# HiLab-git/FPL-plus

Hardware: AMD Instinct MI355X
Metric: 3D volumes/sec (train step, 80x160x160) (higher is better)
Workload: dtype bf16; 1 GPU; UNet3D-DSBN 32-base-ch bf16 (fp32 master weights), per-GPU batch 2x1x80x160x160 synthetic VS crops, DiceLoss + Adam, domain alternating per step; global_batch=2, parallelism=dp1, step=zero_grad+forward+loss+backward+allreduce+adam

## Files before the change

### fpl-plus_amd/csrc/common.h

```cpp
#pragma once
#include <hip/hip_runtime.h>
#include <stdint.h>
#include <stdio.h>
#include <stdarg.h>
#include <string.h>
#include "../../include/fplx.h"

typedef __bf16 bf16_t;

#define FPLX_WAVE 64

inline char* fplx_err_buf() {
  static thread_local char buf[512];
  return buf;
}
inline int fplx_fail(int code, const char* fmt, ...) {
  va_list ap;
  va_start(ap, fmt);
  vsnprintf(fplx_err_buf(), 512, fmt, ap);
  va_end(ap);
  return code;
}
inline int fplx_check_launch(const char* what) {
  hipError_t e = hipGetLastError();
// ... 59 lines not shown
}
struct FplxTileRange { int64_t first, end, step; };
__device__ __forceinline__ FplxTileRange fplx_xcd_tiles(int64_t ntiles, int on) {
  FplxTileRange t = {(int64_t)blockIdx.x, ntiles, (int64_t)gridDim.x};
  if (!on || gridDim.x < 16) return t;
  const unsigned c = blockIdx.x & 7u, xcd = (blockIdx.y * gridDim.x + blockIdx.x) & 7u;
  const int64_t q = ntiles >> 3, r = ntiles & 7;
  const int64_t start = xcd * q + ((int64_t)xcd < r ? xcd : r);
  t.first = start + (blockIdx.x >> 3);
  t.end = start + q + ((int64_t)xcd < r ? 1 : 0);
  t.step = (gridDim.x - c + 7u) >> 3;
  return t;
}
#endif
#define FPLX_KNOB_LIST(X)                                                                                              \
  X(XCD, "xcd", 1)                                                    \
  X(BRICK, "brick", 1)                                    \
  X(BRICK_FILL, "brick_fill", 192)           \
  X(BRICK_GEO, "brick_geo", -1)                    \
  X(BRICK_KSPLIT, "brick_ksplit", 0)                                             \
  X(EDGE_BLOCKS, "edge_blocks", 1024)                             \
  X(STEM_ROWS, "stem_rows", 1)                                              \
  X(OUTCONV_T, "outconv_t", 1)                                 \
  X(OUTCONV_DGRAD_MFMA, "outconv_dgrad_mfma", 1)                                                                       \
  X(OUTCONV_FWD_ROWS, "outconv_fwd_rows", 1)  \
  X(OUTCONV_DGRAD_ROWS, "outconv_dgrad_rows", 1)  \
  X(PACK_TILED, "pack_tiled", 1)                                                                                       \
  X(PACK_MULTI, "pack_multi", 1)                                                                                       \
  X(MARCH, "march", 1)                               \
  X(MARCH64_FW, "march64_fw", 0)                                \
  X(MARCH_DS, "march_ds", 0)                                       \
  X(MARCH128, "march128", 1)                                                                                           \
  X(MARCH64_LW, "march64_lw", 1)            \
  X(MARCH32_V2, "march32_v2", 4)              \
  X(WG_COT_MINVOX, "wg_cot_minvox", 0)                                                                                 \
  X(WG_TW, "wg_tw", 0)                                                                                                 \
  X(WG_CIT, "wg_cit", 2)                                                                                               \
  X(WG_COT, "wg_cot", 2)                                                                                               \
  X(WG_DS, "wg_ds", 0)                                                                                                 \
  X(WG_VOX, "wg_vox", 1)                              \
  X(WG_ROLL, "wg_roll", 1)                     \
  X(WG_ROLL_GEO, "wg_roll_geo", 0)          \
  X(WG_ROLL_M16, "wg_roll_m16", 1)                 \
  X(WG_ROLL_MB, "wg_roll_mb", 1)            \
  X(WG_ROLL_CUS, "wg_roll_cus", 256)                                \
  X(WG_ROLL_OVH, "wg_roll_ovh", 9)                     \
  X(WG_ROLL_MINVOX, "wg_roll_minvox", 0)                                                   \
  X(WG_ROLL2D, "wg_roll2d", 1)              \
  X(WG_ROLL2D_OVH, "wg_roll2d_ovh", 3)      \
  X(WG_REDUCE_ROWS, "wg_reduce_rows", 8)    \
  X(WG_VOX_LW, "wg_vox_lw", 1)              \
  X(WG_VOX_CUS, "wg_vox_cus", 128)          \
  X(WG_VOX_MAXV, "wg_vox_maxv", 10000)         \
  X(STREAM_MIN_W, "stream_min_w", 64)                                                                                  \
  X(TILE_MT, "tile_mt", 0)                                                                                             \
  X(TILE_NT, "tile_nt", 0)                                                                                             \
  X(TILE_KS, "tile_ks", 0)                                                                                             \
  X(MID_TILE, "mid_tile", 1)                                                                                           \
  X(DECONV_ROWS, "deconv_rows", 1)                                                                                     \
  X(DECONV_DGRAD_ROWS, "deconv_dgrad_rows", 1)   \
  X(ROWS_SMALL_DIV, "rows_small_div", 16)   \
  X(EW_GROUP, "ew_group", 1)                                                                                           \
  X(POOL_COL, "pool_col", 1)                         \
  X(EW_INFLIGHT, "ew_inflight", 2)          \
  X(EW_INFLIGHT_REDUCE, "ew_inflight_reduce", 2)
enum FplxKnobId {
#define FPLX_KNOB_ENUM(id, key, def) FPLX_K_##id,
  FPLX_KNOB_LIST(FPLX_KNOB_ENUM)
#undef FPLX_KNOB_ENUM
  FPLX_K_COUNT
};
extern "C" __attribute__((visibility("hidden"))) int64_t fplx_knob_values[FPLX_K_COUNT];
static inline int64_t fplx_knob(int id) { return __atomic_load_n(&fplx_knob_values[id], __ATOMIC_RELAXED); }
static inline int fplx_xcd_on() { return (int)fplx_knob(FPLX_K_XCD); }

static inline int fplx_rows_for(int64_t voxels) {
  constexpr int cap = 512;
  const int div = voxels <= 32768 ? (int)fplx_knob(FPLX_K_ROWS_SMALL_DIV) : 64;
  int64_t r = (voxels + div - 1) / div;
  if (r > cap) r = cap;
  if (r < 1) r = 1;
  return (int)r;
}
```

### fpl-plus_amd/csrc/conv_mfma.hip

```cpp
#include "common.h"
#include <stdlib.h>

namespace {

typedef __attribute__((ext_vector_type(8))) __bf16 bf16x8;
typedef __attribute__((ext_vector_type(16))) float f32x16;

constexpr int DIRECT_THREADS = 256;

template <int MT, int NTL, int MODE>
__global__ void __launch_bounds__(DIRECT_THREADS)
conv_fwd_direct(const bf16_t* __restrict__ x, int64_t ldx, const bf16_t* __restrict__ wp,
                const float* __restrict__ bias, bf16_t* __restrict__ y, int64_t ldy, int N, int D, int H, int W,
                int Cin, int Cout, float* __restrict__ stats, float* __restrict__ partial = nullptr) {
  const int lane = threadIdx.x & 63, wave = threadIdx.x >> 6;
  const int r = lane & 31, kh8 = (lane >> 5) * 8;
  const int64_t V = (int64_t)N * D * H * W;
  const int64_t m0 = ((int64_t)blockIdx.x * 4 + wave) * (MT * 32);
  const int n0 = blockIdx.y * (NTL * 32);

  int vn[MT], vd[MT], vh[MT], vw[MT];
  bool vok[MT];
#pragma unroll
  for (int t = 0; t < MT; ++t) {
// ... 714 lines not shown
#pragma unroll
        for (int g4 = 0; g4 < 4; ++g4)
          *reinterpret_cast<float4*>(out + (tap * 32 + co) * 32 + 8 * g4 + rbase) =
              make_float4(acc[o * 7 + i][4 * g4 + 0], acc[o * 7 + i][4 * g4 + 1], acc[o * 7 + i][4 * g4 + 2],
                          acc[o * 7 + i][4 * g4 + 3]);
      }
    }
  }
}

template <int COT>
__global__ void __launch_bounds__(256)
conv_wgrad_vox(const bf16_t* __restrict__ x, int64_t ldx, const bf16_t* __restrict__ dy, int64_t ldy,
               float* __restrict__ part, int Cin, int Cout, VoxGeo g, int xcd) {
  const FplxBlock bid = fplx_xcd_block(xcd);
  switch (__builtin_amdgcn_readfirstlane(threadIdx.x >> 6)) {
    case 0: wgrad_vox_march<0, COT>(x, ldx, dy, ldy, part, Cin, Cout, g, bid); break;
    case 1: wgrad_vox_march<1, COT>(x, ldx, dy, ldy, part, Cin, Cout, g, bid); break;
    case 2: wgrad_vox_march<2, COT>(x, ldx, dy, ldy, part, Cin, Cout, g, bid); break;
    default: wgrad_vox_march<3, COT>(x, ldx, dy, ldy, part, Cin, Cout, g, bid); break;
  }
}

template <int WV, int SL>
__device__ __forceinline__ void wgrad_vox_lw_chunk(f32x16 (&acc)[7], const char* const (&xb)[7], const char* dyb, const char* mkb) {
  using L = VXL<1>;
  constexpr int NT = (27 - WV + 3) / 4, NKS = VX_KC / 16, NI = NKS * NT;
  constexpr int XOFF = SL * L::X_SLOT, DOFF = SL * L::DY_SLOT, MOFF = SL * L::MK_SLOT;
  constexpr int PD = 3, RING = PD + 1;
  bf16x8 fbw[2], far[RING];
  u32x4v mkr[RING];
  auto masked = [](int j) { const int tap = WV + 4 * j; return ((tap / 3) % 3) != 1 || (tap % 3) != 1; };
  auto load_item = [&](int t) {
    const int ks = t / NT, j = t % NT, tap = WV + 4 * j;
    far[t % RING] = tr_frag(xb[j] + XOFF + ks * 1024);
    if (masked(j)) mkr[t % RING] = *reinterpret_cast<const u32x4v*>(mkb + MOFF + ((tap % 9) * 16 + 2 * ks) * 16);
  };
  fbw[0] = tr_frag(dyb + DOFF);
#pragma unroll
  for (int t = 0; t < PD; ++t) load_item(t);
#pragma unroll
  for (int t = 0; t < NI; ++t) {
    const int ks = t / NT, j = t % NT;
    if (t + PD < NI) load_item(t + PD);
    if (j == 0 && ks + 1 < NKS) fbw[(ks + 1) & 1] = tr_frag(dyb + DOFF + (ks + 1) * 1024);
    __builtin_amdgcn_sched_barrier(0);
    bf16x8 a = far[t % RING];
    if (masked(j)) a = __builtin_bit_cast(bf16x8, __builtin_bit_cast(u32x4v, a) & mkr[t % RING]);
    acc[j] = __builtin_amdgcn_mfma_f32_32x32x16_bf16(a, fbw[ks & 1], acc[j], 0, 0, 0);
    __builtin_amdgcn_sched_barrier(0);
  }
}

template <int WV>
__device__ __forceinline__ void wgrad_vox_lw_compute(float* __restrict__ part, int Cin, int Cout, const VoxGeo& g, const FplxBlock& bid,
                                                     char* smem, int lane, int k0, int k1) {
  using L = VXL<1>;
  const int W = g.W, XR = VX_KC + 2 * W + 2, xplane = XR * 64;
  const int gq = lane >> 4, q = (lane & 15) >> 2, pp = lane & 3;
  const int lane_off = (8 * (gq >> 1) + q) * 64 + (16 * (gq & 1) + 4 * pp) * 2;
  constexpr int NT = (27 - WV + 3) / 4;
  const char* xb[7];
#pragma unroll
  for (int j = 0; j < 7; ++j) {
    const int tap = j < NT ? WV + 4 * j : WV;
    const int kd = tap / 9, kh = (tap / 3) % 3, kw = tap % 3;
    xb[j] = smem + L::X0 + kd * xplane + (kh * W + kw) * 64 + lane_off;
  }
  const char* dyb = smem + L::DY0 + lane_off;
  const char* mkb = smem + L::MK0 + (gq >> 1) * 16;
  f32x16 acc[7];
#pragma unroll
  for (int i = 0; i < 7; ++i)
#pragma unroll
    for (int r = 0; r < 16; ++r) acc[i][r] = 0.f;
  asm volatile("s_waitcnt lgkmcnt(0)\n\ts_barrier" ::: "memory");
  for (int kc = k0;;) {
    wgrad_vox_lw_chunk<WV, 0>(acc, xb, dyb, mkb);
    asm volatile("s_waitcnt lgkmcnt(0)\n\ts_barrier" ::: "memory");
    kc += VX_KC;
    if (kc >= k1) break;
    wgrad_vox_lw_chunk<WV, 1>(acc, xb, dyb, mkb);
    asm volatile("s_waitcnt lgkmcnt(0)\n\ts_barrier" ::: "memory");
    kc += VX_KC;
    if (kc >= k1) break;
  }
  const int ncit = Cin / 32;
  const int cot = bid.y / ncit, cit = bid.y % ncit;
  const int co = lane & 31, rbase = (lane >> 5) * 4;
  const int pair = cot * ncit + cit;
  float* out = part + ((int64_t)bid.x * (ncit * (Cout / 32)) + pair) * (27 * 1024);
#pragma unroll
  for (int i = 0; i < 7; ++i) {
    const int tap = WV + 4 * i;
    if (tap < 27) {
#pragma unroll
      for (int g4 = 0; g4 < 4; ++g4)
        *reinterpret_cast<float4*>(out + (tap * 32 + co) * 32 + 8 * g4 + rbase) =
            make_float4(acc[i][4 * g4 + 0], acc[i][4 * g4 + 1], acc[i][4 * g4 + 2], acc[i][4 * g4 + 3]);
    }
  }
}

__global__ void __launch_bounds__(512)
conv_wgrad_vox_lw(const bf16_t* __restrict__ x, int64_t ldx, const bf16_t* __restrict__ dy, int64_t ldy,
                  float* __restrict__ part, int Cin, int Cout, const VoxGeo g, int xcd) {
  using L = VXL<1>;
  extern __shared__ __attribute__((aligned(16))) char smem[];
  const FplxBlock bid = fplx_xcd_block(xcd);
  const int W = g.W, HW = g.HW, V = g.V;
  const int XR = VX_KC + 2 * W + 2;
  unsigned char* vc = reinterpret_cast<unsigned char*>(smem + L::VC0);
  const int tid = threadIdx.x, lane = tid & 63;
  const int wave8 = __builtin_amdgcn_readfirstlane(tid >> 6);
  const int ncit = Cin / 32;
  const int cot = bid.y / ncit, cit = bid.y % ncit;
  const int k0 = bid.x * g.kper;
  const int k1 = (k0 + g.kper < V) ? k0 + g.kper : V;
  const int halo = HW + W + 1;
  const int tb0 = k0 - halo, tbn = (k1 - k0 + VX_KC - 1) / VX_KC * VX_KC + 2 * halo;
  for (int t = tid; t < tbn; t += 512) {
    const int u = tb0 + t;
    unsigned char c = 0xFF;
    if (u >= 0 && u < V) {
      const unsigned q1 = __umulhi((unsigned)u, g.mW), w_ = (unsigned)u - q1 * (unsigned)W;
      const unsigned q2 = __umulhi(q1, g.mH), h_ = q1 - q2 * (unsigned)g.H;
      const unsigned q3 = __umulhi(q2, g.mD), d_ = q2 - q3 * (unsigned)g.D;
      c = (unsigned char)((d_ == 0 ? 1 : 0) | (d_ == (unsigned)g.D - 1 ? 2 : 0) | (h_ == 0 ? 4 : 0) |
                          (h_ == (unsigned)g.H - 1 ? 8 : 0) | (w_ == 0 ? 16 : 0) | (w_ == (unsigned)W - 1 ? 32 : 0));
    }
    vc[t] = c;
  }
  __syncthreads();
  if (wave8 < 4) {
    switch (wave8) {
      case 0: wgrad_vox_lw_compute<0>(part, Cin, Cout, g, bid, smem, lane, k0, k1); break;
      case 1: wgrad_vox_lw_compute<1>(part, Cin, Cout, g, bid, smem, lane, k0, k1); break;
      case 2: wgrad_vox_lw_compute<2>(part, Cin, Cout, g, bid, smem, lane, k0, k1); break;
      default: wgrad_vox_lw_compute<3>(part, Cin, Cout, g, bid, smem, lane, k0, k1); break;
    }
    return;
  }
  const int lw = wave8 - 4;
  const bf16_t* xg = x + cit * 32;
  const bf16_t* dyg = dy + cot * 32;
  u32x4v rx, ry;
  rx[0] = __builtin_amdgcn_readfirstlane((unsigned)(size_t)xg);
  rx[1] = __builtin_amdgcn_readfirstlane((unsigned)((size_t)xg >> 32) & 0xFFFFu);
  rx[2] = __builtin_amdgcn_readfirstlane((unsigned)((int64_t)V * ldx * 2));
  rx[3] = 0x00020000u;
  ry[0] = __builtin_amdgcn_readfirstlane((unsigned)(size_t)dyg);
  ry[1] = __builtin_amdgcn_readfirstlane((unsigned)((size_t)dyg >> 32) & 0xFFFFu);
  ry[2] = __builtin_amdgcn_readfirstlane((unsigned)((int64_t)V * ldy * 2));
  ry[3] = 0x00020000u;
  const unsigned lds0 = __builtin_amdgcn_readfirstlane((unsigned)(size_t)((__attribute__((address_space(3))) char*)smem));
  auto buf_dma = [&](const u32x4v& rsrc, unsigned vo, unsigned dst_off) {
    const unsigned dst = lds0 + dst_off;
    unsigned keep;
    asm volatile("s_mov_b32 %0, m0\n\ts_mov_b32 m0, %4\n\ts_nop 0\n\tbuffer_load_dwordx4 %1, %2, %3 offen lds\n\ts_mov_b32 m0, %0"
                 : "=&s"(keep) : "v"(vo), "s"(rsrc), "s"(0u), "s"(dst) : "memory");
  };
  const int nxp = (3 * XR + 15) / 16;
  auto stage = [&](int kn, int slot) {
    for (int p = lw; p < nxp + VX_KC / 16; p += 4) {
      if (p < nxp) {
        const int rr = p * 16 + (lane >> 2);
        const int pl = (rr >= XR ? 1 : 0) + (rr >= 2 * XR ? 1 : 0), row = rr - pl * XR;
        const int u = kn + row - (W + 1) + (pl - 1) * HW;
        const int t = u - tb0;
        const bool in = t >= 0 && t < tbn;
        const unsigned c = vc[in ? t : 0];
        const bool ok = in && c != 0xFFu && !((pl == 0 && (c & 2u)) || (pl == 2 && (c & 1u)));
        const unsigned vo = ok ? (unsigned)(((int64_t)u * ldx + (lane & 3) * 8) * 2) : 0x80000000u;
        if (rr < 3 * XR) buf_dma(rx, vo, (unsigned)(L::X0 + slot * L::X_SLOT + p * 1024));
      } else {
        const int v_ = kn + (p - nxp) * 16 + (lane >> 2);
        const unsigned vo = v_ < k1 ? (unsigned)(((int64_t)v_ * ldy + (lane & 3) * 8) * 2) : 0x80000000u;
        buf_dma(ry, vo, (unsigned)(L::DY0 + slot * L::DY_SLOT + (p - nxp) * 1024));
      }
    }
    if (lw < 2) {
      const unsigned c = vc[kn - tb0 + lw * 64 + lane];
      const uint64_t h0 = __ballot(c & 4), h2 = __ballot(c & 8), w0 = __ballot(c & 16), w2 = __ballot(c & 32);
      char* mk_n = smem + L::MK0 + slot * L::MK_SLOT;
#pragma unroll
      for (int rnd = 0; rnd < 2; ++rnd) {
        const int e = rnd * 64 + lane;
        if (e < 72) {
          const int combo = e >> 3, jj = e & 7, kh = combo / 3, kw = combo - 3 * kh;
          const uint64_t inv = (kh == 0 ? h0 : (kh == 2 ? h2 : 0)) | (kw == 0 ? w0 : (kw == 2 ? w2 : 0));
          const unsigned by = (unsigned)(inv >> (8 * jj)) & 0xFFu;
          u32x4v m_;
#pragma unroll
          for (int q_ = 0; q_ < 4; ++q_)
            m_[q_] = ((by >> (2 * q_)) & 1u ? 0u : 0xFFFFu) | ((by >> (2 * q_ + 1)) & 1u ? 0u : 0xFFFF0000u);
          *reinterpret_cast<u32x4v*>(mk_n + (combo * 16 + lw * 8 + jj) * 16) = m_;
        }
      }
    }
  };
  stage(k0, 0);
  asm volatile("s_waitcnt vmcnt(0)" ::: "memory");
  asm volatile("s_waitcnt lgkmcnt(0)\n\ts_barrier" ::: "memory");
  for (int kc = k0, slot = 0;; slot ^= 1) {
    const int kn = kc + VX_KC;
    if (kn < k1) stage(kn, slot ^ 1);
    asm volatile("s_waitcnt vmcnt(0)" ::: "memory");
    asm volatile("s_waitcnt lgkmcnt(0)\n\ts_barrier" ::: "memory");
    kc = kn;
    if (kc >= k1) break;
  }
}

struct VoxCfg { int ok, cot, npairs; VoxGeo g; size_t ws, lds; };
inline VoxCfg vox_cfg(int n, int d, int h, int w, int cin, int cout) {
  VoxCfg c = {};
  const int64_t V = (int64_t)n * d * h * w;
  const int mode = (int)fplx_knob(FPLX_K_WG_VOX);
  if (!mode || cin % 32 != 0 || cout % 32 != 0 || w > VX_MAXW || w < 2 || h < 2 || d < 2 || V >= ((int64_t)1 << 24)) return c;
  if (mode == 1 && V > (int64_t)fplx_knob(FPLX_K_WG_VOX_MAXV)) return c;
  const int lwk = (int)fplx_knob(FPLX_K_WG_VOX_LW);
  const bool lw = lwk == 2 || (lwk == 1 && V <= 2048);
  c.cot = (cout % 64 == 0 && !lw) ? 2 : 1;
  c.npairs = (cin / 32) * (cout / 32);
  const int groups = c.npairs / c.cot;
  const int chunks = (int)((V + VX_KC - 1) / VX_KC);
  const int cus = (int)fplx_knob(FPLX_K_WG_VOX_CUS);
  int S = (cus + groups - 1) / groups;
  if (S > chunks) S = chunks;
  if (S < 1) S = 1;
  const int cper = (chunks + S - 1) / S;
  S = (chunks + cper - 1) / cper;
  VoxGeo& g = c.g;
  g.V = (int)V; g.D = d; g.H = h; g.W = w; g.HW = h * w;
  g.mW = (unsigned)((((uint64_t)1 << 32) + w - 1) / w);
  g.mH = (unsigned)((((uint64_t)1 << 32) + h - 1) / h);
  g.mD = (unsigned)((((uint64_t)1 << 32) + d - 1) / d);
  g.kper = cper * VX_KC; g.S = S;
  c.ws = (size_t)S * c.npairs * 27 * 1024 * sizeof(float);
  c.lds = (size_t)(c.cot == 2 ? VXL<2>::VC0 : VXL<1>::VC0) + (size_t)(g.kper + 2 * (g.HW + w + 1)) + 16;
  c.lds = (c.lds + 15) / 16 * 16;
  if (c.lds > 160 * 1024) return c;
  c.ok = 1;
  return c;
}

__global__ void __launch_bounds__(DIRECT_THREADS)
deconv_fwd_mfma(const bf16_t* __restrict__ x, int64_t ldx, const bf16_t* __restrict__ wf,
                const float* __restrict__ bias, bf16_t* __restrict__ y, int64_t ldy, int N, int D, int H, int W,
                int Cin, int Cout, int sd, int vec_ok, int xcd) {
  const int lane = threadIdx.x & 63, wave = threadIdx.x >> 6;
  const int r = lane & 31, kh8 = (lane >> 5) * 8;
  const int64_t V = (int64_t)N * D * H * W;
  const FplxBlock bid = fplx_xcd_block(xcd);
  const int64_t m0 = ((int64_t)bid.x * 4 + wave) * 32;
  const int n0 = bid.y * 32, tap0 = bid.z * 4;
  const int64_t v = m0 + r;
  const bool ok = v < V;
  const bf16_t* ap = x + (ok ? v : 0) * ldx + kh8;
  const bf16x8 zero = {0, 0, 0, 0, 0, 0, 0, 0};
  f32x16 acc[4];
#pragma unroll
  for (int t = 0; t < 4; ++t)
#pragma unroll
// ... 233 lines not shown
  const int co = lane & 31, rbase = (lane >> 5) * 4;
#pragma unroll
  for (int t = 0; t < 2; ++t)
#pragma unroll
    for (int c = 0; c < CIT; ++c)
#pragma unroll
      for (int i = 0; i < 16; ++i) {
        const int ci = (i & 3) + 8 * (i >> 2) + rbase;
        out[(((2 * wave + t) * CIT + c) * 32 + ci) * 32 + co] = acc[t][c][i];
      }
  if (want_bias) {
    float* red = reinterpret_cast<float*>(smem);
#pragma unroll
    for (int j = 0; j < 8; ++j) red[tid * 8 + j] = bsum[j];
    __syncthreads();
    if (tid < 32) {
      const int cc = tid >> 3, j = tid & 7;
      float t = 0.f;
      for (int k = 0; k < 64; ++k) t += red[(k * 4 + cc) * 8 + j];
      bpart[(int64_t)blockIdx.x * Cout + cot * 32 + tid] = t;
    }
  }
}

__global__ void __launch_bounds__(64) deconv_bias_reduce(const float* __restrict__ bpart, int rows, int C, float* __restrict__ db) {
  const int c = blockIdx.x;
  float t = 0.f;
  for (int r = threadIdx.x; r < rows; r += 64) t += bpart[(int64_t)r * C + c];
  t = wave_sum(t);
  if (threadIdx.x == 0) db[c] = t;
}

__global__ void __launch_bounds__(256)
deconv_wgrad_reduce(const float* __restrict__ part, int nblk, int npairs, int cit, int Cin, int Cout,
                    float* __restrict__ dw, int ntaps) {
  __shared__ float red[256];
  const int64_t per = (int64_t)8 * cit * 1024, total = npairs * per;
  const int64_t i = (int64_t)blockIdx.x * 64 + (threadIdx.x & 63);
  const int pl = threadIdx.x >> 6, o = threadIdx.x & 63;
  float t = 0.f;
  if (i < total)
    for (int b = pl; b < nblk; b += 4) t += part[(int64_t)b * total + i];
  red[pl * 64 + o] = t;
  __syncthreads();
  if (pl != 0 || i >= total) return;
  t = red[o] + red[64 + o] + red[128 + o] + red[192 + o];
  const int co_l = i & 31, ci_l = (i >> 5) & 31, c = (int)((i >> 10) % cit), tap = (int)((i / (1024 * cit)) % 8);
  const int pair = (int)(i / per);
  const int ncig = Cin / (32 * cit);
  const int co = (pair / ncig) * 32 + co_l, ci = ((pair % ncig) * cit + c) * 32 + ci_l;
  if (tap < ntaps) dw[((int64_t)ci * Cout + co) * ntaps + tap] = t;
}

struct DwCfg { int cit, npairs, nblk; size_t ws; };
inline DwCfg dw_cfg(int n, int d, int h, int w, int cin, int cout) {
  DwCfg c;
  c.cit = (cin % 128 == 0) ? 4 : (cin % 64 == 0 ? 2 : 1);
  c.npairs = (cin / (32 * c.cit)) * (cout / 32);
  const int64_t chunks = ((int64_t)n * d * h * w + 127) / 128;
  int nb = 512 / c.npairs;
  if (nb < 1) nb = 1;
  if (nb > chunks) nb = (int)chunks;
  c.nblk = nb;
  c.ws = (size_t)c.nblk * c.npairs * 8 * c.cit * 1024 * sizeof(float) + (size_t)c.nblk * cout * sizeof(float);
  return c;
}

template <int CIN>
struct StreamGeo {
  static constexpr int ROWB = CIN * 2, CH = ROWB / 16;
  static constexpr int SW = 34, SH = 10, SLAB = SW * SH;
  static constexpr int GT = CIN == 32 ? 27 : 3, NG = 27 / GT;
  static constexpr int NSLOT = CIN == 32 ? 4 : 3, NWBUF = NG == 1 ? 1 : 2;
  static constexpr int SLAB_BYTES = SLAB * ROWB, WBUF_BYTES = GT * 32 * ROWB;
  static constexpr int NLD = (SLAB * CH + 255) / 256, NLW = NG == 1 ? 1 : (GT * 32 * CH + 255) / 256;
  static constexpr int LDS = NSLOT * SLAB_BYTES + NWBUF * WBUF_BYTES;
  static __device__ __forceinline__ int swz(int row) { return (row / (16 / CH)) % CH; }
};

template <int CIN>
__global__ void __launch_bounds__(256)
conv_fwd_stream(const bf16_t* __restrict__ x, int64_t ldx, const bf16_t* __restrict__ wp,
                const float* __restrict__ bias, bf16_t* __restrict__ y, int64_t ldy, int N, int D, int H, int W,
                int Cout, float* __restrict__ stats, int tilesH, int tilesW, int dsegs, int dlen) {
  typedef StreamGeo<CIN> G;
  extern __shared__ __attribute__((aligned(16))) char smem[];
  char* slabs = smem;
  char* wbuf = smem + G::NSLOT * G::SLAB_BYTES;
  const int tid = threadIdx.x, lane = tid & 63, wave = tid >> 6;
  const int r = lane & 31, khalf = lane >> 5;
  int b = blockIdx.x;
  const int seg = b % dsegs; b /= dsegs;
  const int tw = b % tilesW; b /= tilesW;
  const int th = b % tilesH; b /= tilesH;
  const int n = b;
  const int h0 = th * 8, w0 = tw * 32, d0 = seg * dlen;
  const int d1 = (d0 + dlen < D) ? d0 + dlen : D;
  const int n0 = blockIdx.y * 32;

  uint4 sreg[G::NLD], wreg[G::NLW];
  auto slab_fetch = [&](int d) {
    const bool dok = d >= 0 && d < D;
#pragma unroll
    for (int k = 0; k < G::NLD; ++k) {
      const int i = tid + k * 256;
      const int vox = i / G::CH, c = i % G::CH;
// ... 827 lines not shown
}
extern "C" int fplx_mfma_conv3d_fwd_act_cat2(const void* x0, const void* x1, int64_t ldx, const void* wp, const float* bias,
                                             const float* slope, void* y, int64_t ldy, int n, int d, int h, int w, int cin,
                                             int cout, int nmod0, hipStream_t st) {
  if (!fplx_mfma_conv3d_act_cat2_ok(n, d, h, w, cin, cout, 0) || !mfma_applicable(ldx, ldy, cin, cout, x0, y, wp)) return 0;
  int geo, ks, bricks;
  fplx_brick_plan(n, d, h, w, cin, cout, &geo, &ks, &bricks);
  return fplx_brick_conv3d_fwd_act(x0, ldx, wp, bias, y, ldy, n, d, h, w, cin, cout, nullptr, nullptr, geo, ks, st, slope, x1, nmod0);
}
extern "C" int fplx_mfma_conv3d_fwd_act(const void* x, int64_t ldx, const void* wp, const float* bias, const float* slope, void* y,
                                        int64_t ldy, int n, int d, int h, int w, int cin, int cout, void* ws, size_t ws_bytes,
                                        int mid, hipStream_t st) {
  return mfma_fwd_impl(x, ldx, wp, bias, y, ldy, n, d, h, w, cin, cout, nullptr, ws, ws_bytes, mid, st, slope);
}

extern "C" int fplx_wgroll_ok(int n, int d, int h, int w, int cin, int cout, int64_t ldx, int64_t ldy);
extern "C" size_t fplx_wgroll_ws_bytes(int n, int d, int h, int w, int cin, int cout);
extern "C" int fplx_wgroll_conv3d_wgrad(const void* x, int64_t ldx, const void* dy, int64_t ldy, float* dw, int n, int d, int h,
                                        int w, int cin, int cout, void* ws, size_t ws_bytes, hipStream_t st, const void* x1, int mid);
extern "C" int fplx_wgrad_reduce_launch(const float* part, int nblk, int npairs, int cin, int cout, float* dw, int mid,
                                        hipStream_t st) {
  const int64_t total = (int64_t)npairs * 27 * 1024;
  wgrad_finish(part, nblk, npairs, cin, cout, dw, mid, st);
  return fplx_check_launch("wgrad_stream_reduce");
}

extern "C" int fplx_mfma_conv3d_wgrad_cit(int n, int d, int h, int w, int cin, int cout) {
  if (cin % 32 != 0 || cout % 32 != 0) return 0;
  return wg_cfg(n, d, h, w, cin, cout).cit;
}

extern "C" size_t fplx_mfma_conv3d_wgrad_ws_bytes(int n, int d, int h, int w, int cin, int cout) {
  if (cin % 32 != 0 || cout % 32 != 0) return 0;
  const size_t a = wg_cfg(n, d, h, w, cin, cout).ws;
  const VoxCfg v = vox_cfg(n, d, h, w, cin, cout);
  size_t m = (v.ok && v.ws > a) ? v.ws : a;
  if (fplx_wgroll_ok(n, d, h, w, cin, cout, cin, cout)) { const size_t r = fplx_wgroll_ws_bytes(n, d, h, w, cin, cout); if (r > m) m = r; }
  return m;
}

extern "C" int fplx_mfma_conv3d_wgrad(const void* x, int64_t ldx, const void* dy, int64_t ldy, float* dw, int n, int d,
                                      int h, int w, int cin, int cout, void* ws, size_t ws_bytes, hipStream_t st,
                                      const void* x1, int mid) {
  if (cin % 32 != 0 || cout % 32 != 0 || ldx % 8 != 0 || ldy % 8 != 0 || ((uintptr_t)x % 16) || ((uintptr_t)dy % 16))
    return 0;
  if (!x1 && !mid) {
    const VoxCfg v = vox_cfg(n, d, h, w, cin, cout);
    if (v.ok) {
      if (ws_bytes < v.ws) return fplx_fail(FPLX_E_WORKSPACE, "mfma_conv3d_wgrad: workspace %zu < %zu", ws_bytes, v.ws);
      dim3 grid(v.g.S, v.npairs / v.cot);
      const int lwk = (int)fplx_knob(FPLX_K_WG_VOX_LW);
      if ((lwk == 2 || (lwk == 1 && v.g.V <= 2048)) && v.cot == 1 && (int64_t)v.g.V * ldx * 2 < ((int64_t)1 << 31) &&
          (int64_t)v.g.V * ldy * 2 < ((int64_t)1 << 31)) {
        (void)hipFuncSetAttribute((const void*)conv_wgrad_vox_lw, hipFuncAttributeMaxDynamicSharedMemorySize, (int)v.lds);
        conv_wgrad_vox_lw<<<grid, 512, v.lds, st>>>((const bf16_t*)x, ldx, (const bf16_t*)dy, ldy, (float*)ws, cin, cout, v.g, fplx_xcd_on());
      } else if (v.cot == 2) {
        (void)hipFuncSetAttribute((const void*)conv_wgrad_vox<2>, hipFuncAttributeMaxDynamicSharedMemorySize, (int)v.lds);
        conv_wgrad_vox<2><<<grid, 256, v.lds, st>>>((const bf16_t*)x, ldx, (const bf16_t*)dy, ldy, (float*)ws, cin, cout, v.g, fplx_xcd_on());
      } else {
        (void)hipFuncSetAttribute((const void*)conv_wgrad_vox<1>, hipFuncAttributeMaxDynamicSharedMemorySize, (int)v.lds);
        conv_wgrad_vox<1><<<grid, 256, v.lds, st>>>((const bf16_t*)x, ldx, (const bf16_t*)dy, ldy, (float*)ws, cin, cout, v.g, fplx_xcd_on());
      }
      wgrad_finish((const float*)ws, v.g.S, v.npairs, cin, cout, dw, 0, st);
      int rcv = fplx_check_launch("mfma_conv3d_wgrad_vox");
      return rcv < 0 ? rcv : 1;
    }
  }
  {
    const int rr = fplx_wgroll_conv3d_wgrad(x, ldx, dy, ldy, dw, n, d, h, w, cin, cout, ws, ws_bytes, st, x1, mid);
    if (rr != 0) return rr;
  }
  const WgCfg c = wg_cfg(n, d, h, w, cin, cout);
  if (x1 && (c.cit != 2 || cin != 64 || ((uintptr_t)x1 % 16))) return 0;
  if (ws_bytes < c.ws) return fplx_fail(FPLX_E_WORKSPACE, "mfma_conv3d_wgrad: workspace %zu < %zu", ws_bytes, c.ws);
  dim3 grid(c.nblk, c.npairs / (c.cit * c.cot));
#define LAUNCH_WG2(TW_, CIT_, COT_, TWOD_)                                                                          \
  do {                                                                                                              \
    const size_t lds = (size_t)(3 * CIT_ * (WG_TH + 2) * (TW_ + 2) + COT_ * WG_TH * TW_) * 64;                      \
    (void)hipFuncSetAttribute((const void*)conv_wgrad_stream<TW_, CIT_, COT_, TWOD_>, hipFuncAttributeMaxDynamicSharedMemorySize, (int)lds); \
    conv_wgrad_stream<TW_, CIT_, COT_, TWOD_><<<grid, 256, lds, st>>>((const bf16_t*)x, ldx, (const bf16_t*)dy, ldy, (float*)ws, n, d, \
                                                                h, w, cin, cout, c.tilesH, c.tilesW, c.dsegs, c.dlen, (const bf16_t*)x1, fplx_xcd_on()); \
  } while (0)
#define LAUNCH_WG(TW_, CIT_, COT_) do { if (mid) LAUNCH_WG2(TW_, CIT_, COT_, true); else LAUNCH_WG2(TW_, CIT_, COT_, false); } while (0)
  if (c.tw == 32) { if (c.cot == 2) LAUNCH_WG(32, 1, 2); else if (c.cit == 2) LAUNCH_WG(32, 2, 1); else LAUNCH_WG(32, 1, 1); }
  else { if (c.cot == 2) LAUNCH_WG(16, 1, 2); else if (c.cit == 2) LAUNCH_WG(16, 2, 1); else LAUNCH_WG(16, 1, 1); }
#undef LAUNCH_WG
#undef LAUNCH_WG2
  const int64_t total = (int64_t)c.npairs * 27 * 1024;
  wgrad_finish((const float*)ws, c.nblk, c.npairs, cin, cout, dw, mid, st);
  int rc = fplx_check_launch("mfma_conv3d_wgrad");
  return rc < 0 ? rc : 1;
}

extern "C" int fplx_mfma_deconv2_fwd(const void* x, int64_t ldx, const void* wf, const float* bias, void* y, int64_t ldy,
                                     int n, int d, int h, int w, int cin, int cout, int sd, hipStream_t st) {
  if (cin % 32 != 0 || cout % 32 != 0 || ldx % 8 != 0 || ((uintptr_t)x % 16) || ((uintptr_t)wf % 16)) return 0;
  const int64_t V = (int64_t)n * d * h * w;
  if (V >= ((int64_t)1 << 31)) return 0;
  const int vec_ok = ldy % 8 == 0 && ((uintptr_t)y % 16) == 0;
  {
    const int krows = (int)fplx_knob(FPLX_K_DECONV_ROWS);
    const int ks = cin / 16, ntc = cout / 32;
    if (krows && sd == 2 && vec_ok && V >= 32 * 1024 && ((ks == 4 && ntc == 1) || (ks == 8 && ntc == 2) || (ks == 8 && ntc == 1) ||
                                                         (ks == 4 && ntc == 2))) {
      const int64_t nt = (V + 31) / 32;
      const unsigned nb = (unsigned)(nt < 1024 ? nt : 1024);
#define LAUNCH_DR(KS_, NTC_) deconv_fwd_rows<KS_, NTC_><<<nb, 256, 0, st>>>((const bf16_t*)x, ldx, (const bf16_t*)wf, bias, \
                                                                           (bf16_t*)y, ldy, n, d, h, w, fplx_xcd_on())
// ... 34 lines not shown
  if (sd == 2 && fplx_knob(FPLX_K_DECONV_DGRAD_ROWS) && ((V + 127) / 128) * (cin / 64) < 128 && cin % 64 == 0 && cout % 16 == 0 &&
      ldx % 8 == 0 && ((uintptr_t)dx % 16) == 0) {
    dim3 gs((unsigned)((V + 31) / 32), cin / 64);
    deconv_dgrad_small<<<gs, 256, 0, st>>>((const bf16_t*)dy, ldy, (const bf16_t*)wb, (bf16_t*)dx, ldx, n, d, h, w, cout, cin);
    int rcs = fplx_check_launch("mfma_deconv2_dgrad_small");
    return rcs < 0 ? rcs : 1;
  }
#define LAUNCH_DD(MT_, NTL_, MODE_, GRID_)                                                                          \
  conv_fwd_direct<MT_, NTL_, MODE_><<<GRID_, DIRECT_THREADS, 0, st>>>((const bf16_t*)dy, ldy, (const bf16_t*)wb, nullptr, \
                                                                      (bf16_t*)dx, ldx, n, d, h, w, cout, cin, nullptr)
  if (cin % 64 == 0) {
    dim3 grid((unsigned)((V + 255) / 256), cin / 64);
    if ((int64_t)grid.x * grid.y < 192) {
      dim3 g1((unsigned)((V + 127) / 128), cin / 64);
      if (sd == 2) LAUNCH_DD(1, 2, 1, g1); else LAUNCH_DD(1, 2, 2, g1);
    } else if (sd == 2) LAUNCH_DD(2, 2, 1, grid);
    else LAUNCH_DD(2, 2, 2, grid);
  } else {
    dim3 grid((unsigned)((V + 511) / 512), cin / 32);
    if (sd == 2) LAUNCH_DD(4, 1, 1, grid); else LAUNCH_DD(4, 1, 2, grid);
  }
#undef LAUNCH_DD
  int rc = fplx_check_launch("mfma_deconv2_dgrad");
  return rc < 0 ? rc : 1;
}

extern "C" size_t fplx_mfma_deconv2_wgrad_ws_bytes(int n, int d, int h, int w, int cin, int cout) {
  if (cin % 32 != 0 || cout % 32 != 0) return 0;
  return dw_cfg(n, d, h, w, cin, cout).ws;
}

extern "C" int fplx_mfma_deconv2_wgrad(const void* x, int64_t ldx, const void* dy, int64_t ldy, float* dw, float* db,
                                       int n, int d, int h, int w, int cin, int cout, void* ws, size_t ws_bytes,
                                       int sd, hipStream_t st) {
  if (cin % 32 != 0 || cout % 32 != 0 || ldx % 8 != 0 || ldy % 8 != 0 || ((uintptr_t)x % 16) || ((uintptr_t)dy % 16))
    return 0;
  const DwCfg c = dw_cfg(n, d, h, w, cin, cout);
  if (ws_bytes < c.ws) return fplx_fail(FPLX_E_WORKSPACE, "mfma_deconv2_wgrad: workspace %zu < %zu", ws_bytes, c.ws);
  dim3 grid(c.nblk, c.npairs);
  const size_t lds = (size_t)(c.cit + 8) * 128 * 64;
  float* bpart = db ? (float*)((char*)ws + (size_t)c.nblk * c.npairs * 8 * c.cit * 1024 * sizeof(float)) : nullptr;
#define LAUNCH_DW(CIT)                                                                                              \
  do {                                                                                                              \
    (void)hipFuncSetAttribute((const void*)deconv_wgrad_mfma<CIT>, hipFuncAttributeMaxDynamicSharedMemorySize, (int)lds); \
    deconv_wgrad_mfma<CIT><<<grid, 256, lds, st>>>((const bf16_t*)x, ldx, (const bf16_t*)dy, ldy, (float*)ws, bpart, n, d, \
                                                   h, w, cin, cout, sd);                                            \
  } while (0)
  if (c.cit == 4) LAUNCH_DW(4);
  else if (c.cit == 2) LAUNCH_DW(2);
  else LAUNCH_DW(1);
#undef LAUNCH_DW
  const int64_t total = (int64_t)c.npairs * 8 * c.cit * 1024;
  if (db) deconv_bias_reduce<<<cout, 64, 0, st>>>(bpart, c.nblk, cout, db);
  deconv_wgrad_reduce<<<(unsigned)((total + 63) / 64), 256, 0, st>>>((const float*)ws, c.nblk, c.npairs, c.cit, cin, cout, dw,
                                                                      4 * sd);
  int rc = fplx_check_launch("mfma_deconv2_wgrad");
  return rc < 0 ? rc : 1;
}
```

Baseline: 246.9 volumes/s.

## Write vox wgrad directly to dw, add deep wgrad kernel and row-wise deconv reduce

When there is a single split (S==1), the lightweight vox wgrad kernel now transposes its accumulators through LDS and writes the final weight layout straight into dw. This skips the partial-buffer write and the separate wgrad_finish pass. A new 8-wave conv_wgrad_deep kernel for the cot==2 case is added behind knob level 2, so it is off by default. The deconv wgrad reduction is replaced by a row-per-block kernel that reduces float4 partials across blocks in LDS and writes coalesced rows. The cost is more LDS per block for the direct path, plus extra code complexity.

```diff
diff --git a/fpl-plus_amd/csrc/common.h b/fpl-plus_amd/csrc/common.h
--- a/fpl-plus_amd/csrc/common.h
+++ b/fpl-plus_amd/csrc/common.h
@@ -135,6 +135,7 @@
   X(WG_VOX_LW, "wg_vox_lw", 1)              \
   X(WG_VOX_CUS, "wg_vox_cus", 128)          \
   X(WG_VOX_MAXV, "wg_vox_maxv", 10000)         \
+  X(WG_DEEP, "wg_deep", 1)                  \
   X(STREAM_MIN_W, "stream_min_w", 64)                                                                                  \
   X(TILE_MT, "tile_mt", 0)                                                                                             \
   X(TILE_NT, "tile_nt", 0)                                                                                             \
diff --git a/fpl-plus_amd/csrc/conv_mfma.hip b/fpl-plus_amd/csrc/conv_mfma.hip
--- a/fpl-plus_amd/csrc/conv_mfma.hip
+++ b/fpl-plus_amd/csrc/conv_mfma.hip
@@ -790,7 +790,25 @@
   }
 }
 
-template <int WV>
+constexpr int VXD_TS = 1024 + 4;
+__device__ __forceinline__ void wgrad_vox_direct_copy(const char* smem, float* __restrict__ dw, int Cin, const FplxBlock& bid, int tid) {
+  const float* tile = reinterpret_cast<const float*>(smem);
+  const int ncit = Cin / 32;
+  const int cot = bid.y / ncit, cit = bid.y % ncit;
+  float* row0 = dw + ((int64_t)cot * 32 * Cin + cit * 32) * 27;
+#pragma unroll 1
+  for (int i = tid; i < 32 * 216; i += 512) {
+    const int row = i / 216, j = i - row * 216;
+    float v[4];
+#pragma unroll
+    for (int k = 0; k < 4; ++k) {
+      const int e = 4 * j + k, ci = e / 27, tap = e - 27 * ci;
+      v[k] = tile[tap * VXD_TS + row * 32 + ci];
+    }
+    *reinterpret_cast<float4*>(row0 + (int64_t)row * Cin * 27 + 4 * j) = make_float4(v[0], v[1], v[2], v[3]);
+  }
+}
+template <int WV, bool DIRECT>
 __device__ __forceinline__ void wgrad_vox_lw_compute(float* __restrict__ part, int Cin, int Cout, const VoxGeo& g, const FplxBlock& bid,
                                                      char* smem, int lane, int k0, int k1) {
   using L = VXL<1>;
@@ -823,6 +841,23 @@
     kc += VX_KC;
     if (kc >= k1) break;
   }
+  if constexpr (DIRECT) {
+    float* tile = reinterpret_cast<float*>(smem);
+    const int co = lane & 31, rbase = (lane >> 5) * 4;
+#pragma unroll
+    for (int i = 0; i < 7; ++i) {
+      const int tap = WV + 4 * i;
+      if (tap < 27) {
+#pragma unroll
+        for (int g4 = 0; g4 < 4; ++g4)
+          *reinterpret_cast<float4*>(tile + tap * VXD_TS + co * 32 + 8 * g4 + rbase) =
+              make_float4(acc[i][4 * g4 + 0], acc[i][4 * g4 + 1], acc[i][4 * g4 + 2], acc[i][4 * g4 + 3]);
+      }
+    }
+    asm volatile("s_waitcnt lgkmcnt(0)\n\ts_barrier" ::: "memory");
+    wgrad_vox_direct_copy(smem, part, Cin, bid, WV * 64 + lane);
+    return;
+  }
   const int ncit = Cin / 32;
   const int cot = bid.y / ncit, cit = bid.y % ncit;
   const int co = lane & 31, rbase = (lane >> 5) * 4;
@@ -840,6 +875,7 @@
   }
 }
 
+template <bool DIRECT>
 __global__ void __launch_bounds__(512)
 conv_wgrad_vox_lw(const bf16_t* __restrict__ x, int64_t ldx, const bf16_t* __restrict__ dy, int64_t ldy,
                   float* __restrict__ part, int Cin, int Cout, const VoxGeo g, int xcd) {
@@ -872,10 +908,10 @@
   __syncthreads();
   if (wave8 < 4) {
     switch (wave8) {
-      case 0: wgrad_vox_lw_compute<0>(part, Cin, Cout, g, bid, smem, lane, k0, k1); break;
-      case 1: wgrad_vox_lw_compute<1>(part, Cin, Cout, g, bid, smem, lane, k0, k1); break;
-      case 2: wgrad_vox_lw_compute<2>(part, Cin, Cout, g, bid, smem, lane, k0, k1); break;
-      default: wgrad_vox_lw_compute<3>(part, Cin, Cout, g, bid, smem, lane, k0, k1); break;
+      case 0: wgrad_vox_lw_compute<0, DIRECT>(part, Cin, Cout, g, bid, smem, lane, k0, k1); break;
+      case 1: wgrad_vox_lw_compute<1, DIRECT>(part, Cin, Cout, g, bid, smem, lane, k0, k1); break;
+      case 2: wgrad_vox_lw_compute<2, DIRECT>(part, Cin, Cout, g, bid, smem, lane, k0, k1); break;
+      default: wgrad_vox_lw_compute<3, DIRECT>(part, Cin, Cout, g, bid, smem, lane, k0, k1); break;
     }
     return;
   }
@@ -948,6 +984,208 @@
     kc = kn;
     if (kc >= k1) break;
   }
+  if constexpr (DIRECT) {
+    asm volatile("s_waitcnt lgkmcnt(0)\n\ts_barrier" ::: "memory");
+    wgrad_vox_direct_copy(smem, part, Cin, bid, tid);
+  }
+}
+
+template <int WV> struct VXD {
+  static constexpr int COMBO = WV < 4 ? WV : WV + 1, NT = WV < 6 ? 4 : 3;
+  static constexpr int CO_C = WV & 1;
+  static constexpr int tap(int j) { return j < 3 ? 9 * j + COMBO : 4 + 9 * (WV >> 1); }
+};
+
+template <int WV, int SL>
+__device__ __forceinline__ void wgrad_deep_chunk(f32x16 (&acc)[7], const char* const (&xb)[4], const char* dyb, const char* mkb) {
+  using L = VXL<2>;
+  using T = VXD<WV>;
+  constexpr int NKS = VX_KC / 16, DYPLANE = VX_KC * 64;
+  constexpr int XOFF = SL * L::X_SLOT, DOFF = SL * L::DY_SLOT, MOFF = SL * L::MK_SLOT;
+  bf16x8 fa[4], fb[2][2];
+  u32x4v mk[2];
+  fb[0][0] = tr_frag(dyb + DOFF);
+  fb[0][1] = tr_frag(dyb + DOFF + DYPLANE);
+  mk[0] = *reinterpret_cast<const u32x4v*>(mkb + MOFF + (T::COMBO * 16) * 16);
+#pragma unroll
+  for (int j = 0; j < T::NT; ++j) fa[j] = tr_frag(xb[j] + XOFF);
+#pragma unroll
+  for (int ks = 0; ks < NKS; ++ks) {
+    const int b = ks & 1;
+    if (ks + 1 < NKS) {
+      fb[b ^ 1][0] = tr_frag(dyb + DOFF + (ks + 1) * 1024);
+      fb[b ^ 1][1] = tr_frag(dyb + DOFF + DYPLANE + (ks + 1) * 1024);
+      mk[b ^ 1] = *reinterpret_cast<const u32x4v*>(mkb + MOFF + (T::COMBO * 16 + 2 * (ks + 1)) * 16);
+    }
+#pragma unroll
+    for (int j = 0; j < T::NT; ++j) {
+      __builtin_amdgcn_sched_barrier(0);
+      bf16x8 a = fa[j];
+      if (j < 3) a = __builtin_bit_cast(bf16x8, __builtin_bit_cast(u32x4v, a) & mk[b]);
+      if (j < 3) {
+        acc[j] = __builtin_amdgcn_mfma_f32_32x32x16_bf16(a, fb[b][0], acc[j], 0, 0, 0);
+        acc[3 + j] = __builtin_amdgcn_mfma_f32_32x32x16_bf16(a, fb[b][1], acc[3 + j], 0, 0, 0);
+      } else {
+        acc[6] = __builtin_amdgcn_mfma_f32_32x32x16_bf16(a, fb[b][T::CO_C], acc[6], 0, 0, 0);
+      }
+      if (ks + 1 < NKS) fa[j] = tr_frag(xb[j] + XOFF + (ks + 1) * 1024);
+    }
+    __builtin_amdgcn_sched_barrier(0);
+  }
+}
+
+template <int WV>
+__device__ __forceinline__ void wgrad_deep_wave(const bf16_t* __restrict__ x, int64_t ldx, const bf16_t* __restrict__ dy, int64_t ldy,
+                                                float* __restrict__ part, int Cin, int Cout, const VoxGeo& g, const FplxBlock& bid,
+                                                char* smem, int lane, int k0, int k1, int tb0, int tbn) {
+  using L = VXL<2>;
+  using T = VXD<WV>;
+  const int W = g.W, HW = g.HW, V = g.V;
+  const int XR = VX_KC + 2 * W + 2, xplane = XR * 64;
+  const unsigned char* vc = reinterpret_cast<const unsigned char*>(smem + L::VC0);
+  const int ncit = Cin / 32;
+  const int cot = bid.y / ncit, cit = bid.y % ncit;
+  const bf16_t* xg = x + cit * 32;
+  const bf16_t* dyg = dy + cot * 64;
+  u32x4v rx, ry;
+  rx[0] = __builtin_amdgcn_readfirstlane((unsigned)(size_t)xg);
+  rx[1] = __builtin_amdgcn_readfirstlane((unsigned)((size_t)xg >> 32) & 0xFFFFu);
+  rx[2] = __builtin_amdgcn_readfirstlane((unsigned)((int64_t)V * ldx * 2));
+  rx[3] = 0x00020000u;
+  ry[0] = __builtin_amdgcn_readfirstlane((unsigned)(size_t)dyg);
+  ry[1] = __builtin_amdgcn_readfirstlane((unsigned)((size_t)dyg >> 32) & 0xFFFFu);
+  ry[2] = __builtin_amdgcn_readfirstlane((unsigned)((int64_t)V * ldy * 2));
+  ry[3] = 0x00020000u;
+  const unsigned lds0 = __builtin_amdgcn_readfirstlane((unsigned)(size_t)((__attribute__((address_space(3))) char*)smem));
+  auto buf_dma = [&](const u32x4v& rsrc, unsigned vo, unsigned dst_off) {
+    const unsigned dst = lds0 + dst_off;
+    unsigned keep;
+    asm volatile("s_mov_b32 %0, m0\n\ts_mov_b32 m0, %4\n\ts_nop 0\n\tbuffer_load_dwordx4 %1, %2, %3 offen lds\n\ts_mov_b32 m0, %0"
+                 : "=&s"(keep) : "v"(vo), "s"(rsrc), "s"(0u), "s"(dst) : "memory");
+  };
+  const int nxp = (3 * XR + 15) / 16;
+  auto stage = [&](int kn, int slot) {
+    for (int p = WV; p < nxp + 2 * (VX_KC / 16); p += 8) {
+      if (p < nxp) {
+        const int rr = p * 16 + (lane >> 2);
+        const int pl = (rr >= XR ? 1 : 0) + (rr >= 2 * XR ? 1 : 0), row = rr - pl * XR;
+        const int u = kn + row - (W + 1) + (pl - 1) * HW;
+        const int t = u - tb0;
+        const bool in = t >= 0 && t < tbn;
+        const unsigned c = vc[in ? t : 0];
+        const bool ok = in && c != 0xFFu && !((pl == 0 && (c & 2u)) || (pl == 2 && (c & 1u)));
+        const unsigned vo = ok ? (unsigned)(((int64_t)u * ldx + (lane & 3) * 8) * 2) : 0x80000000u;
+        if (rr < 3 * XR) buf_dma(rx, vo, (unsigned)(L::X0 + slot * L::X_SLOT + p * 1024));
+      } else {
+        const int q = p - nxp, o = q / (VX_KC / 16), piece = q % (VX_KC / 16);
+        const int v_ = kn + piece * 16 + (lane >> 2);
+        const unsigned vo = v_ < k1 ? (unsigned)(((int64_t)v_ * ldy + o * 32 + (lane & 3) * 8) * 2) : 0x80000000u;
+        buf_dma(ry, vo, (unsigned)(L::DY0 + slot * L::DY_SLOT + o * (VX_KC * 64) + piece * 1024));
+      }
+    }
+    if (WV < 2) {
+      const unsigned c = vc[kn - tb0 + WV * 64 + lane];
+      const uint64_t h0 = __ballot(c & 4), h2 = __ballot(c & 8), w0 = __ballot(c & 16), w2 = __ballot(c & 32);
+      char* mk_n = smem + L::MK0 + slot * L::MK_SLOT;
+#pragma unroll
+      for (int rnd = 0; rnd < 2; ++rnd) {
+        const int e = rnd * 64 + lane;
+        if (e < 72) {
+          const int combo = e >> 3, jj = e & 7, kh = combo / 3, kw = combo - 3 * kh;
+          const uint64_t inv = (kh == 0 ? h0 : (kh == 2 ? h2 : 0)) | (kw == 0 ? w0 : (kw == 2 ? w2 : 0));
+          const unsigned by = (unsigned)(inv >> (8 * jj)) & 0xFFu;
+          u32x4v m_;
+#pragma unroll
+          for (int q_ = 0; q_ < 4; ++q_)
+            m_[q_] = ((by >> (2 * q_)) & 1u ? 0u : 0xFFFFu) | ((by >> (2 * q_ + 1)) & 1u ? 0u : 0xFFFF0000u);
+          *reinterpret_cast<u32x4v*>(mk_n + (combo * 16 + WV * 8 + jj) * 16) = m_;
+        }
+      }
+    }
+  };
+  const int gq = lane >> 4, q = (lane & 15) >> 2, pp = lane & 3;
+  const int lane_off = (8 * (gq >> 1) + q) * 64 + (16 * (gq & 1) + 4 * pp) * 2;
+  const char* xb[4];
+#pragma unroll
+  for (int j = 0; j < 4; ++j) {
+    const int tap = T::tap(j < T::NT ? j : 0);
+    const int kd = tap / 9, kh = (tap / 3) % 3, kw = tap % 3;
+    xb[j] = smem + L::X0 + kd * xplane + (kh * W + kw) * 64 + lane_off;
+  }
+  const char* dyb = smem + L::DY0 + lane_off;
+  const char* mkb = smem + L::MK0 + (gq >> 1) * 16;
+  f32x16 acc[7];
+#pragma unroll
+  for (int i = 0; i < 7; ++i)
+#pragma unroll
+    for (int r = 0; r < 16; ++r) acc[i][r] = 0.f;
+  stage(k0, 0);
+  asm volatile("s_waitcnt vmcnt(0) lgkmcnt(0)\n\ts_barrier" ::: "memory");
+  for (int kc = k0;;) {
+    if (kc + VX_KC < k1) stage(kc + VX_KC, 1);
+    wgrad_deep_chunk<WV, 0>(acc, xb, dyb, mkb);
+    asm volatile("s_waitcnt vmcnt(0) lgkmcnt(0)\n\ts_barrier" ::: "memory");
+    kc += VX_KC;
+    if (kc >= k1) break;
+    if (kc + VX_KC < k1) stage(kc + VX_KC, 0);
+    wgrad_deep_chunk<WV, 1>(acc, xb, dyb, mkb);
+    asm volatile("s_waitcnt vmcnt(0) lgkmcnt(0)\n\ts_barrier" ::: "memory");
+    kc += VX_KC;
+    if (kc >= k1) break;
+  }
+  const int co = lane & 31, rbase = (lane >> 5) * 4;
+#pragma unroll
+  for (int o = 0; o < 2; ++o) {
+    const int pair = (cot * 2 + o) * ncit + cit;
+    float* out = part + ((int64_t)bid.x * (ncit * (Cout / 32)) + pair) * (27 * 1024);
+#pragma unroll
+    for (int j = 0; j < T::NT; ++j) {
+      if (j == 3 && o != T::CO_C) continue;
+      const int tap = T::tap(j), i = j < 3 ? o * 3 + j : 6;
+#pragma unroll
+      for (int g4 = 0; g4 < 4; ++g4)
+        *reinterpret_cast<float4*>(out + (tap * 32 + co) * 32 + 8 * g4 + rbase) =
+            make_float4(acc[i][4 * g4 + 0], acc[i][4 * g4 + 1], acc[i][4 * g4 + 2], acc[i][4 * g4 + 3]);
+    }
+  }
+}
+
+__global__ void __launch_bounds__(512)
+conv_wgrad_deep(const bf16_t* __restrict__ x, int64_t ldx, const bf16_t* __restrict__ dy, int64_t ldy,
+                float* __restrict__ part, int Cin, int Cout, const VoxGeo g, int xcd) {
+  using L = VXL<2>;
+  extern __shared__ __attribute__((aligned(16))) char smem[];
+  const FplxBlock bid = fplx_xcd_block(xcd);
+  const int W = g.W, HW = g.HW, V = g.V;
+  unsigned char* vc = reinterpret_cast<unsigned char*>(smem + L::VC0);
+  const int tid = threadIdx.x, lane = tid & 63;
+  const int k0 = bid.x * g.kper;
+  const int k1 = (k0 + g.kper < V) ? k0 + g.kper : V;
+  const int halo = HW + W + 1;
+  const int tb0 = k0 - halo, tbn = (k1 - k0 + VX_KC - 1) / VX_KC * VX_KC + 2 * halo;
+  for (int t = tid; t < tbn; t += 512) {
+    const int u = tb0 + t;
+    unsigned char c = 0xFF;
+    if (u >= 0 && u < V) {
+      const unsigned q1 = __umulhi((unsigned)u, g.mW), w_ = (unsigned)u - q1 * (unsigned)W;
+      const unsigned q2 = __umulhi(q1, g.mH), h_ = q1 - q2 * (unsigned)g.H;
+      const unsigned q3 = __umulhi(q2, g.mD), d_ = q2 - q3 * (unsigned)g.D;
+      c = (unsigned char)((d_ == 0 ? 1 : 0) | (d_ == (unsigned)g.D - 1 ? 2 : 0) | (h_ == 0 ? 4 : 0) |
+                          (h_ == (unsigned)g.H - 1 ? 8 : 0) | (w_ == 0 ? 16 : 0) | (w_ == (unsigned)W - 1 ? 32 : 0));
+    }
+    vc[t] = c;
+  }
+  __syncthreads();
+  switch (__builtin_amdgcn_readfirstlane(tid >> 6)) {
+    case 0: wgrad_deep_wave<0>(x, ldx, dy, ldy, part, Cin, Cout, g, bid, smem, lane, k0, k1, tb0, tbn); break;
+    case 1: wgrad_deep_wave<1>(x, ldx, dy, ldy, part, Cin, Cout, g, bid, smem, lane, k0, k1, tb0, tbn); break;
+    case 2: wgrad_deep_wave<2>(x, ldx, dy, ldy, part, Cin, Cout, g, bid, smem, lane, k0, k1, tb0, tbn); break;
+    case 3: wgrad_deep_wave<3>(x, ldx, dy, ldy, part, Cin, Cout, g, bid, smem, lane, k0, k1, tb0, tbn); break;
+    case 4: wgrad_deep_wave<4>(x, ldx, dy, ldy, part, Cin, Cout, g, bid, smem, lane, k0, k1, tb0, tbn); break;
+    case 5: wgrad_deep_wave<5>(x, ldx, dy, ldy, part, Cin, Cout, g, bid, smem, lane, k0, k1, tb0, tbn); break;
+    case 6: wgrad_deep_wave<6>(x, ldx, dy, ldy, part, Cin, Cout, g, bid, smem, lane, k0, k1, tb0, tbn); break;
+    default: wgrad_deep_wave<7>(x, ldx, dy, ldy, part, Cin, Cout, g, bid, smem, lane, k0, k1, tb0, tbn); break;
+  }
 }
 
 struct VoxCfg { int ok, cot, npairs; VoxGeo g; size_t ws, lds; };
@@ -1287,6 +1525,58 @@
   if (tap < ntaps) dw[((int64_t)ci * Cout + co) * ntaps + tap] = t;
 }
 
+__global__ void __launch_bounds__(1024)
+deconv_wgrad_reduce_rows(const float* __restrict__ part, int nblk, int npairs, int cit, int Cin, int Cout,
+                         float* __restrict__ dw, int ntaps) {
+  __shared__ float4 red[16 * 64];
+  __shared__ __attribute__((aligned(16))) float tile[256];
+  const int PL = blockDim.x >> 6;
+  const int o = threadIdx.x & 63, pl = threadIdx.x >> 6;
+  const int tap = o >> 3, co4 = o & 7;
+  const int r = blockIdx.x;
+  const int ci_l = r & 31, c = (r >> 5) % cit, pair = r / (32 * cit);
+  const int64_t per = (int64_t)8 * cit * 1024, total = npairs * per;
+  const bool live = tap < ntaps;
+  float4 t = make_float4(0.f, 0.f, 0.f, 0.f);
+  if (live) {
+    const float* p = part + pair * per + ((tap * cit + c) * 32 + ci_l) * 32 + co4 * 4;
+    int b = pl;
+    for (; b + 3 * PL < nblk; b += 4 * PL) {
+      const float4 v0 = *reinterpret_cast<const float4*>(p + (int64_t)b * total);
+      const float4 v1 = *reinterpret_cast<const float4*>(p + (int64_t)(b + PL) * total);
+      const float4 v2 = *reinterpret_cast<const float4*>(p + (int64_t)(b + 2 * PL) * total);
+      const float4 v3 = *reinterpret_cast<const float4*>(p + (int64_t)(b + 3 * PL) * total);
+      t.x += v0.x; t.y += v0.y; t.z += v0.z; t.w += v0.w;
+      t.x += v1.x; t.y += v1.y; t.z += v1.z; t.w += v1.w;
+      t.x += v2.x; t.y += v2.y; t.z += v2.z; t.w += v2.w;
+      t.x += v3.x; t.y += v3.y; t.z += v3.z; t.w += v3.w;
+    }
+    for (; b < nblk; b += PL) {
+      const float4 v = *reinterpret_cast<const float4*>(p + (int64_t)b * total);
+      t.x += v.x; t.y += v.y; t.z += v.z; t.w += v.w;
+    }
+  }
+  red[pl * 64 + o] = t;
+  __syncthreads();
+  if (pl == 0 && live) {
+    for (int k = 1; k < PL; ++k) {
+      const float4 q = red[k * 64 + o];
+      t.x += q.x; t.y += q.y; t.z += q.z; t.w += q.w;
+    }
+    tile[(4 * co4 + 0) * ntaps + tap] = t.x;
+    tile[(4 * co4 + 1) * ntaps + tap] = t.y;
+    tile[(4 * co4 + 2) * ntaps + tap] = t.z;
+    tile[(4 * co4 + 3) * ntaps + tap] = t.w;
+  }
+  __syncthreads();
+  if (threadIdx.x < 8 * ntaps) {
+    const int ncig = Cin / (32 * cit);
+    const int co0 = (pair / ncig) * 32, ci = ((pair % ncig) * cit + c) * 32 + ci_l;
+    *reinterpret_cast<float4*>(dw + ((int64_t)ci * Cout + co0) * ntaps + 4 * threadIdx.x) =
+        *reinterpret_cast<const float4*>(tile + 4 * threadIdx.x);
+  }
+}
+
 struct DwCfg { int cit, npairs, nblk; size_t ws; };
 inline DwCfg dw_cfg(int n, int d, int h, int w, int cin, int cout) {
   DwCfg c;
@@ -2220,8 +2510,19 @@
       const int lwk = (int)fplx_knob(FPLX_K_WG_VOX_LW);
       if ((lwk == 2 || (lwk == 1 && v.g.V <= 2048)) && v.cot == 1 && (int64_t)v.g.V * ldx * 2 < ((int64_t)1 << 31) &&
           (int64_t)v.g.V * ldy * 2 < ((int64_t)1 << 31)) {
-        (void)hipFuncSetAttribute((const void*)conv_wgrad_vox_lw, hipFuncAttributeMaxDynamicSharedMemorySize, (int)v.lds);
-        conv_wgrad_vox_lw<<<grid, 512, v.lds, st>>>((const bf16_t*)x, ldx, (const bf16_t*)dy, ldy, (float*)ws, cin, cout, v.g, fplx_xcd_on());
+        if (fplx_knob(FPLX_K_WG_DEEP) && fplx_knob(FPLX_K_WG_VOX) == 1 && v.g.S == 1 && ((uintptr_t)dw % 16) == 0) {
+          const size_t ldsd = v.lds > (size_t)27 * VXD_TS * 4 ? v.lds : (size_t)27 * VXD_TS * 4;
+          (void)hipFuncSetAttribute((const void*)conv_wgrad_vox_lw<true>, hipFuncAttributeMaxDynamicSharedMemorySize, (int)ldsd);
+          conv_wgrad_vox_lw<true><<<grid, 512, ldsd, st>>>((const bf16_t*)x, ldx, (const bf16_t*)dy, ldy, dw, cin, cout, v.g, fplx_xcd_on());
+          int rcd = fplx_check_launch("mfma_conv3d_wgrad_vox_lw_direct");
+          return rcd < 0 ? rcd : 1;
+        }
+        (void)hipFuncSetAttribute((const void*)conv_wgrad_vox_lw<false>, hipFuncAttributeMaxDynamicSharedMemorySize, (int)v.lds);
+        conv_wgrad_vox_lw<false><<<grid, 512, v.lds, st>>>((const bf16_t*)x, ldx, (const bf16_t*)dy, ldy, (float*)ws, cin, cout, v.g, fplx_xcd_on());
+      } else if (v.cot == 2 && fplx_knob(FPLX_K_WG_DEEP) >= 2 && fplx_knob(FPLX_K_WG_VOX) == 1 &&
+                 (int64_t)v.g.V * ldx * 2 < ((int64_t)1 << 31) && (int64_t)v.g.V * ldy * 2 < ((int64_t)1 << 31)) {
+        (void)hipFuncSetAttribute((const void*)conv_wgrad_deep, hipFuncAttributeMaxDynamicSharedMemorySize, (int)v.lds);
+        conv_wgrad_deep<<<grid, 512, v.lds, st>>>((const bf16_t*)x, ldx, (const bf16_t*)dy, ldy, (float*)ws, cin, cout, v.g, fplx_xcd_on());
       } else if (v.cot == 2) {
         (void)hipFuncSetAttribute((const void*)conv_wgrad_vox<2>, hipFuncAttributeMaxDynamicSharedMemorySize, (int)v.lds);
         conv_wgrad_vox<2><<<grid, 256, v.lds, st>>>((const bf16_t*)x, ldx, (const bf16_t*)dy, ldy, (float*)ws, cin, cout, v.g, fplx_xcd_on());
@@ -2362,8 +2663,14 @@
 #undef LAUNCH_DW
   const int64_t total = (int64_t)c.npairs * 8 * c.cit * 1024;
   if (db) deconv_bias_reduce<<<cout, 64, 0, st>>>(bpart, c.nblk, cout, db);
-  deconv_wgrad_reduce<<<(unsigned)((total + 63) / 64), 256, 0, st>>>((const float*)ws, c.nblk, c.npairs, c.cit, cin, cout, dw,
-                                                                      4 * sd);
+  if (fplx_knob(FPLX_K_WG_DEEP) && ((uintptr_t)dw % 16) == 0) {
+    const int plw = c.nblk > 256 ? 16 : (c.nblk > 128 ? 8 : (c.nblk > 16 ? 4 : (c.nblk > 1 ? 2 : 1)));
+    deconv_wgrad_reduce_rows<<<(unsigned)(c.npairs * c.cit * 32), 64 * plw, 0, st>>>((const float*)ws, c.nblk, c.npairs, c.cit, cin,
+                                                                                       cout, dw, 4 * sd);
+  } else {
+    deconv_wgrad_reduce<<<(unsigned)((total + 63) / 64), 256, 0, st>>>((const float*)ws, c.nblk, c.npairs, c.cit, cin, cout, dw,
+                                                                        4 * sd);
+  }
   int rc = fplx_check_launch("mfma_deconv2_wgrad");
   return rc < 0 ? rc : 1;
 }
```

New measurement: 248.7 volumes/s, median of 6. About the same (+0.7%).
